# avi2924/Speech-Intent-Recognizer

Hardware: AMD Instinct MI355X
Metric: utterances/sec (16 kHz, 3 s clips), inference: HIP STFT+mel+CNN/BiGRU forward + argmax (higher is better)
Workload: dtype f32

## Files before the change

### speech-intent-recognizer_amd/csrc/conv_wino2_f16x3_kernel.h

```cpp
#pragma once
#include "conv_wino_bf16x6_kernel.h"
#include "wino2_geo.h"

constexpr int W2_RS = 11;
constexpr int W2_NPOS = 18 * W2_RS;
constexpr int W2_RAW_PIECES = (W2_NPOS * 4 + 63) / 64;
constexpr int W2_RAW_BYTES = W2_RAW_PIECES * 1024;
constexpr int W2_PLB = 16 * 1024;
constexpr int W2_NRAW = 3;
constexpr int W2_V_BYTES = 2 * W2_PLB;
constexpr int W2_XCH_BYTES = 3 * W2_PLB;
constexpr int W2_LDS_BYTES = 2 * W2_V_BYTES + W2_NRAW * W2_RAW_BYTES + W2_XCH_BYTES;
constexpr int W2_THREADS = 768;
constexpr int W2_PPW = (W2_RAW_PIECES + 3) / 4;

__device__ __forceinline__ int w2_div(int n, const W2Div& d) {
    const unsigned un = (unsigned)n;
    if (d.pow2) return (int)(un >> d.sh);
    const unsigned t = __umulhi(d.m, un);
    return (int)((t + ((un - t) >> 1)) >> d.sh);
}

__device__ __forceinline__ void split_w_f16x3(float u, unsigned short& p0, unsigned short& p1, unsigned int* status) {
    constexpr float LIM = 31.984375f;
// ... 8 lines not shown
                                                            unsigned int* status) {
    const int total = cin * 16 * cout;
    if (idx >= total) return;
    const int e = idx & 15, co = (idx >> 4) % cout, g = (idx >> 4) / cout;
    const int ci = (g / 16) * 16 + e, f = g % 16, i = f >> 2, j = f & 3;
    const float* gk = w + ((size_t)co * cin + ci) * 9;
    const float Gm[4][3] = {{1.f, 0.f, 0.f}, {.5f, .5f, .5f}, {.5f, -.5f, .5f}, {0.f, 0.f, 1.f}};
    float u = 0.0f;
#pragma unroll
    for (int k = 0; k < 3; ++k) {
        float t = 0.0f;
#pragma unroll
        for (int l = 0; l < 3; ++l) t = fmaf(gk[k * 3 + l], Gm[j][l], t);
        u = fmaf(Gm[i][k], t, u);
    }
    if (j == 3) u = -u;
    split_w_f16x3(u, wpb[idx], wpb[(size_t)total + idx], status);
}
#ifndef SIR_NO_STANDALONE_KERNELS
static __global__ void prep_conv_w_wino_f16x3_kernel(const float* __restrict__ w, unsigned short* __restrict__ wpb, int cin, int cout,
                                                     unsigned int* status) {
    prep_conv_w_wino_f16x3_elem(w, wpb, cin, cout, blockIdx.x * blockDim.x + threadIdx.x, status);
}
#endif
__device__ __forceinline__ void prep_conv_wT_wino_f16x3_elem(const float* __restrict__ w, unsigned short* __restrict__ wpb, int cin_f, int cout_f,
                                                             int idx, unsigned int* status) {
    const int total = cout_f * 16 * cin_f;
    if (idx >= total) return;
    const int e = idx & 15, cop = (idx >> 4) % cin_f, g = (idx >> 4) / cin_f;
    const int co_f = (g / 16) * 16 + e, f = g % 16, i = f >> 2, j = f & 3;
    const float* gk = w + ((size_t)co_f * cin_f + cop) * 9;
    const float Gm[4][3] = {{1.f, 0.f, 0.f}, {.5f, .5f, .5f}, {.5f, -.5f, .5f}, {0.f, 0.f, 1.f}};
    float u = 0.0f;
#pragma unroll
    for (int k = 0; k < 3; ++k) {
        float t = 0.0f;
#pragma unroll
        for (int l = 0; l < 3; ++l) t = fmaf(gk[8 - (k * 3 + l)], Gm[j][l], t);
        u = fmaf(Gm[i][k], t, u);
    }
    if (j == 3) u = -u;
    split_w_f16x3(u, wpb[idx], wpb[(size_t)total + idx], status);
}
#ifndef SIR_NO_STANDALONE_KERNELS
static __global__ void prep_conv_wT_wino_f16x3_kernel(const float* __restrict__ w, unsigned short* __restrict__ wpb, int cin_f, int cout_f,
                                                       unsigned int* status) {
    prep_conv_wT_wino_f16x3_elem(w, wpb, cin_f, cout_f, blockIdx.x * blockDim.x + threadIdx.x, status);
}
#endif

typedef float w2_f32x4 __attribute__((ext_vector_type(4)));
typedef unsigned w2_u32x2 __attribute__((ext_vector_type(2)));
__device__ __forceinline__ void w2_barrier() { asm volatile("s_waitcnt lgkmcnt(0)\n\ts_barrier" ::: "memory"); }
__device__ __forceinline__ void w2_read_row(unsigned base, w2_f32x4& r0, w2_f32x4& r1, w2_f32x4& r2, w2_f32x4& r3) {
    asm volatile("ds_read_b128 %0, %4\n\tds_read_b128 %1, %4 offset:64\n\tds_read_b128 %2, %4 offset:128\n\tds_read_b128 %3, %4 offset:192"
                 : "=&v"(r0), "=&v"(r1), "=&v"(r2), "=&v"(r3) : "v"(base) : "memory");
}
template <int OFF>
__device__ __forceinline__ void w2_write64(unsigned base, uint2 v) {
    const w2_u32x2 d = {v.x, v.y};
    asm volatile("ds_write_b64 %0, %1 offset:%2" :: "v"(base), "v"(d), "n"(OFF) : "memory");
}

__device__ long long w2_dbg_stamps[2][32];
__device__ long long w2_dbg_fine[8][8];
template <int CIN, int COUT, int OUT_MODE, int DBG = 0, int PRIO = 3, bool RAGGED = false>
__global__ __launch_bounds__(W2_THREADS, 3) void conv3x3_wino2_f16x3_kernel(
    const float* __restrict__ x, const unsigned short* __restrict__ wpb, const float* __restrict__ scale,
    const float* __restrict__ shift, float* __restrict__ out, Wino2Geo geo, float2* __restrict__ stats, const float* __restrict__ zeros) {
    constexpr int NCH = CIN / 16, G = NCH * 16, NCHO = COUT >= 64 ? COUT / 64 : 1;
    static_assert(CIN % 16 == 0 && (COUT % 64 == 0 || COUT == 32), "16-channel chunks; 64-channel tasks (32: the n = 1 consumer waves only keep the barriers)");
    static_assert(NCH >= 2, "a task's exchange pieces are read behind its closing barrier; the next task's are written >= one barrier later");
    extern __shared__ __attribute__((aligned(1024))) unsigned char w2s[];
    constexpr int VB = W2_V_BYTES;
    unsigned char* const vbuf = w2s;
    unsigned char* const rawbuf = w2s + 2 * VB;
    unsigned char* const xchbuf = rawbuf + W2_NRAW * W2_RAW_BYTES;

    const int tid = threadIdx.x, lane = tid & 63, wv = __builtin_amdgcn_readfirstlane(tid >> 6);
    const bool producer = wv < 4;
    const int H = geo.H, W = geo.W, TW = geo.TW, NG = geo.NG, RBN = geo.RBN;
    const int* const ctab = OUT_MODE <= 1 ? geo.ctab : nullptr;
    const int NS = ctab ? RBN * ctab[0] : geo.NS;
    const int ntask_s = (NS - (int)blockIdx.x + (int)gridDim.x - 1) / (int)gridDim.x;
    const int ntask = ntask_s * NCHO;
    if (ntask <= 0) return;
    const int nsteps = ntask * NCH;

    auto task_geo = [&](int lt, int& g0, int& ty0, int& ch, int& s) {
        s = (int)blockIdx.x + (lt / NCHO) * (int)gridDim.x;
        ch = lt % NCHO;
        const int cb = w2_div(s, geo.dRBN), rb = s - cb * RBN;
        g0 = ctab ? ctab[1 + cb] : 4 * cb; ty0 = 8 * rb;
    };
    constexpr bool IDLE_DMA = COUT < 64;
    constexpr int D_STRIDE = 4, D_PPW = (W2_RAW_PIECES + D_STRIDE - 1) / D_STRIDE;
    const int d_stride = D_STRIDE;
    const int d_rank = producer ? wv : ((wv - 4) >> 1);
    int pre_lr[D_PPW], pre_lc[D_PPW], pre_part[D_PPW];
#pragma unroll
    for (int ii = 0; ii < D_PPW; ++ii) {
        const int slot = 64 * (d_rank + d_stride * ii) + lane, pos = slot >> 2, sp = slot & 3;
        const int lr = pos / W2_RS;
        const int lc = pos - lr * W2_RS - ((lr >> 1) & 1);
        const bool hole = lr > 17 || lc < 0 || lc > 9;
        pre_lr[ii] = hole ? (1 << 20) : lr;
        pre_lc[ii] = lc;
        pre_part[ii] = (sp ^ (((lr >> 2) & 1) << 1)) * 4;
    }
    auto raw_offsets = [&](int g0, int ty0, unsigned (&off)[D_PPW]) {
        const int gimg = ctab ? w2_div(g0, geo.dTW) : 0;
        const int plo = ctab ? 2 * TW * gimg : 0, phi = ctab ? plo + (RAGGED ? min(W, geo.wtab[gimg] >> geo.wsh) : W) : 2 * NG;
#pragma unroll
        for (int ii = 0; ii < D_PPW; ++ii) {
            const int gy = 2 * ty0 - 1 + pre_lr[ii];
            const int P = 2 * g0 - 1 + pre_lc[ii];
            const int Pc = min(max(P, 0), 2 * NG - 1);
            const int bb = w2_div(Pc, geo.d2TW), px = Pc - bb * 2 * TW;
            const bool ok = gy >= 0 && gy < H && P >= plo && P < phi && px < W;
            off[ii] = ok ? (unsigned)(((bb * H + gy) * W + px) * CIN + pre_part[ii]) : ~0u;
        }
    };
        auto raw_issue = [&](const unsigned (&off)[D_PPW], int c, int slot_buf) {
#pragma unroll
        for (int ii = 0; ii < D_PPW; ++ii) {
            const int k = d_rank + d_stride * ii;
            if (k < W2_RAW_PIECES) {
                const float* src = off[ii] == ~0u ? zeros : x + off[ii];
                __builtin_amdgcn_global_load_lds((sir_gptr_t)(src + c * 16), (sir_lptr_t)(rawbuf + slot_buf * W2_RAW_BYTES + k * 1024), 16, 0, 0);
            }
        }
    };
    int ig0, ity0, ich, is_;
    unsigned roff[D_PPW];
    int roff_task = -1;
    auto issue_chunk = [&](int q) {
        if (q >= nsteps) return;
        const int lt = q / NCH, c = q - lt * NCH;
        if (lt != roff_task) { task_geo(lt, ig0, ity0, ich, is_); raw_offsets(ig0, ity0, roff); roff_task = lt; }
        raw_issue(roff, c, q % W2_NRAW);
    };
    int nst = 0;
    auto stamp = [&]() {
        if (DBG && blockIdx.x == 0 && lane == 0 && (wv == 0 || wv == 4) && nst < 32) w2_dbg_stamps[producer ? 0 : 1][nst] = __builtin_amdgcn_s_memtime();
        ++nst;
    };

    if (producer) {
        if (PRIO) __builtin_amdgcn_s_setprio(PRIO);
        __builtin_amdgcn_s_setreg((1 ) | (23 << 6) | (0 << 11), 1);
        const int wg = wv;
        const int tR = wg >> 1, tH = wg & 1, tm = lane >> 1, tP1 = lane & 1;
        const int tty = tm & 7, ttx = tm >> 3, tpart = 2 * tH + tP1;
        unsigned ra_rel[3];
#pragma unroll
        for (int rr = 0; rr < 3; ++rr) {
            const int lr = 2 * tty + tR + rr;
            ra_rel[rr] = (unsigned)((lr * W2_RS + 2 * ttx + ((lr >> 1) & 1)) * 64 + ((tpart ^ (((lr >> 2) & 1) << 1)) * 16));
        }
        const unsigned raw_a = (unsigned)(uintptr_t)rawbuf, v_a = (unsigned)(uintptr_t)vbuf + (8 * tR) * 1024 + tH * 512 + tm * 16 + tP1 * 8;
        if (!IDLE_DMA) {
            issue_chunk(0);
            issue_chunk(1);
            asm volatile("s_waitcnt vmcnt(0)" ::: "memory");
        }
        w2_barrier();
        bool edge = false, z0 = false, z3 = false;
        auto fine = [&](int s_, int k_) {
            if (DBG && blockIdx.x == 0 && lane == 0 && wv == 0 && s_ >= 8 && s_ < 16) w2_dbg_fine[s_ - 8][k_] = __builtin_amdgcn_s_memtime();
        };
#pragma unroll 1
        for (int s = 0; s <= nsteps; ++s) {
            stamp();
            fine(s, 0);
            if (s < nsteps) {
                if (!IDLE_DMA && !(DBG & 2)) issue_chunk(s + 2);
                fine(s, 1);
                if (s % NCH == 0) {
                    int cg0, cty0, cch, cs;
                    task_geo(s / NCH, cg0, cty0, cch, cs);
                    const int t0 = cg0 - w2_div(cg0, geo.dTW) * TW;
                    edge = !ctab && (t0 == 0 || t0 + 3 >= TW - 1);
                    const int txx = (t0 + ttx) - w2_div(t0 + ttx, geo.dTW) * TW;
                    z0 = txx == 0; z3 = txx == TW - 1;
                }
                const unsigned rb = raw_a + (s % W2_NRAW) * W2_RAW_BYTES, vd = v_a + (s & 1) * VB;
                if (!(DBG & 4)) {
                w2_f32x4 q[3][4];
#pragma unroll
                for (int rr = 0; rr < 3; ++rr) w2_read_row(rb + ra_rel[rr], q[rr][0], q[rr][1], q[rr][2], q[rr][3]);
                asm volatile("s_waitcnt lgkmcnt(0)" ::: "memory");
                fine(s, 2);
                if (edge) {
                    asm volatile("" ::: "memory");
                    const w2_f32x4 zero4 = {0.0f, 0.0f, 0.0f, 0.0f};
#pragma unroll
                    for (int rr = 0; rr < 3; ++rr) { q[rr][0] = z0 ? zero4 : q[rr][0]; q[rr][3] = z3 ? zero4 : q[rr][3]; }
                }
                auto rows = [&](auto trc) {
                    constexpr int TR = decltype(trc)::value;
#pragma unroll
                    for (int il = 0; il < 2; ++il) {
                        w2_f32x4 R[4];
#pragma unroll
                        for (int j = 0; j < 4; ++j) {
                            if (TR == 0) R[j] = il == 0 ? q[0][j] - q[2][j] : q[1][j] + q[2][j];
                            else         R[j] = il == 0 ? q[1][j] - q[0][j] : q[0][j] - q[2][j];
                        }
                        const w2_f32x4 V[4] = {R[0] - R[2], R[1] + R[2], R[2] - R[1], R[1] - R[3]};
#pragma unroll
                        for (int j = 0; j < 4; ++j) {
                            const unsigned d = vd + (4 * il + j) * 1024;
                            uint2 sh, sl;
                            split2h_pair_ovfl(V[j].x, V[j].y, sh.x, sl.x);
                            split2h_pair_ovfl(V[j].z, V[j].w, sh.y, sl.y);
                            w2_write64<0>(d, sh);
                            w2_write64<W2_PLB>(d, sl);
                        }
                    }
                };
                if (tR == 0) rows(std::integral_constant<int, 0>{});
                else rows(std::integral_constant<int, 1>{});
                if (DBG) asm volatile("s_waitcnt lgkmcnt(0)" ::: "memory");
                fine(s, 3);
                }
                if (!IDLE_DMA) {
                    if (s + 2 < nsteps) asm volatile("s_waitcnt vmcnt(%0)" :: "n"(W2_RAW_PIECES / 4) : "memory");
                    else asm volatile("s_waitcnt vmcnt(0)" ::: "memory");
                }
            }
            stamp();
            fine(s, 4);
            w2_barrier();
            fine(s, 5);
        }
        return;
    }

    const int cw = wv - 4, mn = cw & 1, mi = cw >> 1, m = lane & 31, h = lane >> 5;
    if (COUT < 64 && mn == 1) {
        if (IDLE_DMA) {
            if (!(DBG & 2)) { issue_chunk(0); issue_chunk(1); }
            asm volatile("s_waitcnt vmcnt(0)" ::: "memory");
            w2_barrier();
#pragma unroll 1
            for (int s = 0; s <= nsteps; ++s) {
                if (s < nsteps) {
                    if (!(DBG & 2)) issue_chunk(s + 2);
                    if (s + 2 < nsteps) asm volatile("s_waitcnt vmcnt(%0)" :: "n"(W2_RAW_PIECES / 4) : "memory");
                    else asm volatile("s_waitcnt vmcnt(0)" ::: "memory");
                }
                w2_barrier();
            }
            return;
        }
        w2_barrier();
        w2_barrier();
        for (int lt = 0; lt < ntask; ++lt)
            for (int c = 0; c < NCH; ++c) w2_barrier();
        return;
    }
    const unsigned wlane = (unsigned)((m * 2 + h) * 16);
    const unsigned char* const wbase = reinterpret_cast<const unsigned char*>(wpb) + (size_t)mn * 1024;
    constexpr int NPW = 2;
    uint4 wq[4][NPW];
    auto load_w = [&](int gidx, int chh, uint4 (&q)[NPW]) {
#pragma unroll
        for (int p = 0; p < NPW; ++p)
            q[p] = *reinterpret_cast<const uint4*>(wbase + ((size_t)(p * G + gidx) * (COUT * 2) + (size_t)chh * 128) * 16 + wlane);
    };
    int g0, ty0, ch, s_idx;
    task_geo(0, g0, ty0, ch, s_idx);
#pragma unroll
    for (int j = 0; j < 4; ++j) load_w(4 * mi + j, ch, wq[j]);
    f32x16 acc[4];
#pragma unroll
    for (int j = 0; j < 4; ++j)
#pragma unroll
        for (int r = 0; r < 16; ++r) acc[j][r] = 0.0f;
    w2_barrier();
    float run_s[NCHO], run_q[NCHO];
#pragma unroll
    for (int k = 0; k < NCHO; ++k) { run_s[k] = 0.0f; run_q[k] = 0.0f; }

    stamp();
    stamp();
    w2_barrier();
#pragma unroll 1
    for (int lt = 0; lt < ntask; ++lt) {
        int g0n = g0, ty0n = ty0, chn = ch, sn = s_idx;
        if (lt + 1 < ntask) task_geo(lt + 1, g0n, ty0n, chn, sn);
#pragma unroll 1
        for (int c = 0; c < NCH; ++c) {
            stamp();
            const int sc = lt * NCH + c;
            const bool task_end = c == NCH - 1;
            const unsigned char* abase = vbuf + (sc & 1) * VB + h * 512 + m * 16 + (4 * mi) * 1024;
            const int gnxt = (task_end ? 0 : c + 1) * 16 + 4 * mi;
#pragma unroll
            for (int jp = 0; jp < 2; ++jp) {
                constexpr int NPA = 2;
                bf16x8 a[2][NPA], bq[2][3];
#pragma unroll
                for (int jj = 0; jj < 2; ++jj) {
#pragma unroll
                    for (int p = 0; p < NPA; ++p)
                        a[jj][p] = __builtin_bit_cast(bf16x8, *reinterpret_cast<const uint4*>(abase + p * W2_PLB + (2 * jp + jj) * 1024));
                    const f16x8 uh = __builtin_bit_cast(f16x8, wq[2 * jp + jj][0]);
                    bq[jj][0] = __builtin_bit_cast(bf16x8, uh);
                    bq[jj][1] = __builtin_bit_cast(bf16x8, uh * (_Float16)2048.0f);
                    bq[jj][2] = __builtin_bit_cast(bf16x8, wq[2 * jp + jj][1]);
                }
                if (DBG & 8) {
#pragma unroll
                    for (int jj = 0; jj < 2; ++jj)
                        acc[2 * jp + jj][0] += __builtin_bit_cast(float4, a[jj][0]).x + __builtin_bit_cast(float4, a[jj][1]).y + __builtin_bit_cast(float4, a[jj][NPA - 1]).z +
                                               __builtin_bit_cast(float4, bq[jj][0]).x + __builtin_bit_cast(float4, bq[jj][1]).y + __builtin_bit_cast(float4, bq[jj][2]).z;
                } else {
                    constexpr int HA[3] = {1, 0, 0}, HB[3] = {0, 2, 1};
#pragma unroll
                    for (int t3 = 0; t3 < 3; ++t3)
#pragma unroll
                        for (int jj = 0; jj < 2; ++jj)
                            acc[2 * jp + jj] = __builtin_amdgcn_mfma_f32_32x32x16_f16(__builtin_bit_cast(f16x8, a[jj][HA[t3]]),
                                                                                      __builtin_bit_cast(f16x8, bq[jj][HB[t3]]), acc[2 * jp + jj], 0, 0, 0);
                }
#pragma unroll
                for (int jj = 0; jj < 2; ++jj) if (!(DBG & 64)) load_w(gnxt + 2 * jp + jj, task_end ? chn : ch, wq[2 * jp + jj]);
                __builtin_amdgcn_sched_barrier(0);
            }
            stamp();
            if (!task_end) w2_barrier();
        }
        if (DBG & 16) { w2_barrier(); if (acc[0][0] == 1234.5f && acc[1][1] + acc[2][2] + acc[3][3] == 4.0f) out[0] = 1.0f; }
        else {
            {
                float4* const xch = reinterpret_cast<float4*>(xchbuf);
                float own[2][4];
#pragma unroll
                for (int b = 0; b < 2; ++b) {
                    const f32x16 Wc = b == 0 ? acc[0] + acc[1] + acc[2] : acc[1] - acc[2] + acc[3];
#pragma unroll
                    for (int k = 0; k < 4; ++k) {
                        if (k == mi) {
#pragma unroll
                            for (int e = 0; e < 4; ++e) own[b][e] = Wc[4 * k + e];
                        } else {
                            float4* dst = xch + (size_t)((mn * 4 + mi) * 3 + ((k - mi - 1) & 3)) * 128 + lane;
                            dst[b * 64] = make_float4(Wc[4 * k], Wc[4 * k + 1], Wc[4 * k + 2], Wc[4 * k + 3]);
                        }
                    }
                }
                w2_barrier();
                float Y[2][2][4];
#pragma unroll
                for (int i = 0; i < 4; ++i) {
                    const int kk = (mi - i - 1) & 3;
                    const float4* src = xch + (size_t)((mn * 4 + i) * 3 + (kk < 3 ? kk : 0)) * 128 + lane;
#pragma unroll
                    for (int b = 0; b < 2; ++b) {
                        const float4 v = src[b * 64];
                        const float w[4] = {i == mi ? own[b][0] : v.x, i == mi ? own[b][1] : v.y, i == mi ? own[b][2] : v.z, i == mi ? own[b][3] : v.w};
#pragma unroll
                        for (int e = 0; e < 4; ++e) {
                            if (i == 0) Y[0][b][e] = w[e];
                            else if (i <= 2) Y[0][b][e] += w[e];
                            if (i == 1) Y[1][b][e] = w[e];
                            else if (i >= 2) Y[1][b][e] -= w[e];
                        }
                    }
                }
                const int co = ch * 64 + mn * 32 + m;
                float ssum = 0.0f, ssq = 0.0f;
                float sc_ = 1.0f, sh_ = 0.0f;
                constexpr float DESC = H3_LO_INV;
                if (OUT_MODE <= 1) { sc_ = scale[co] * DESC; sh_ = shift[co]; }
                {
                    const int gc = g0 + mi;
                    const int img = w2_div(gc, geo.dTW), tx = gc - img * TW;
                    const bool tvalid = gc < (ctab ? (w2_div(g0, geo.dTW) + 1) * TW : NG);
                    const int wpi = RAGGED ? min(geo.Wp, geo.wtab[w2_div(g0, geo.dTW)] >> (geo.wsh + 1)) : geo.Wp;
                    if (OUT_MODE <= 1) {
                        float pooled[4];
#pragma unroll
                        for (int e = 0; e < 4; ++e) {
                            float v = 0.0f;
#pragma unroll
                            for (int a = 0; a < 2; ++a)
#pragma unroll
                                for (int b = 0; b < 2; ++b) v = fmaxf(v, fmaf(Y[a][b][e], sc_, sh_));
                            pooled[e] = v;
                        }
                        if (tvalid && tx < wpi) {
                            if (OUT_MODE == 0) {
#pragma unroll
                                for (int e = 0; e < 4; ++e)
                                    out[(((size_t)img * geo.Hp + ty0 + 4 * h + e) * geo.Wp + tx) * COUT + co] = pooled[e];
                            } else {
                                const size_t oidx = ((size_t)img * geo.Wp + tx) * (COUT * geo.Hp) + (size_t)co * geo.Hp + ty0 + 4 * h;
                                const float4 v4 = make_float4(pooled[0], pooled[1], pooled[2], pooled[3]);
                                *reinterpret_cast<float4*>(out + oidx) = v4;
                                if (stats) {
                                    unsigned short* planes = reinterpret_cast<unsigned short*>(stats);
                                    const size_t plane = (size_t)geo.B * geo.Wp * (COUT * geo.Hp);
                                    uint2 hh, ll;
                                    split2h_quad(v4, hh, ll);
                                    *reinterpret_cast<uint2*>(planes + oidx) = hh;
                                    *reinterpret_cast<uint2*>(planes + plane + oidx) = ll;
                                }
                            }
                        }
                    } else {
#pragma unroll
                        for (int e = 0; e < 4; ++e)
#pragma unroll
                            for (int a = 0; a < 2; ++a)
#pragma unroll
                                for (int b = 0; b < 2; ++b) {
                                    const int gy = 2 * (ty0 + 4 * h + e) + a, gx = 2 * tx + b;
                                    if (tvalid && gx < W) {
                                        const float v = Y[a][b][e] * DESC;
                                        out[(((size_t)img * H + gy) * W + gx) * COUT + co] = v;
                                        ssum += v;
                                        ssq = fmaf(v, v, ssq);
                                    }
                                }
                    }
                }
                if (OUT_MODE == 2) {
#pragma unroll
                    for (int k = 0; k < NCHO; ++k)
                        if (k == ch) { run_s[k] += ssum; run_q[k] += ssq; }
                }
            }
        }
        g0 = g0n; ty0 = ty0n; ch = chn; s_idx = sn;
#pragma unroll
        for (int j = 0; j < 4; ++j)
#pragma unroll
            for (int r = 0; r < 16; ++r) acc[j][r] = 0.0f;
    }
    if (OUT_MODE == 2 && stats) {
#pragma unroll
        for (int k = 0; k < NCHO; ++k) {
            float a = run_s[k], q = run_q[k];
            a += __shfl_xor(a, 32);
            q += __shfl_xor(q, 32);
            if (h == 0) stats[((size_t)blockIdx.x * 4 + mi) * COUT + k * 64 + mn * 32 + m] = make_float2(a, q);
        }
    }
}

template <int CIN, int COUT, int OUT_MODE, int DBG = 0, int PRIO = 3, bool RAGGED = false>
static inline hipError_t launch_conv_wino2(hipStream_t st, Wino2Geo g, const float* x, const unsigned short* wpb, const float* scale,
                                           const float* shift, float* out, float2* stats, const float* zeros, int max_wg = 256,
                                           const int* ctab = nullptr, int ncol_max = 0, const int* wtab = nullptr, int wsh = 0) {
    if (RAGGED && (!ctab || !wtab)) return hipErrorInvalidValue;
    g.wtab = wtab; g.wsh = wsh;
    if (ctab) {
        if (OUT_MODE > 1 || ncol_max < 1) return hipErrorInvalidValue;
        g.ctab = ctab;
        g.NS = g.RBN * ncol_max;
    }
    const int nwg = g.NS < max_wg ? g.NS : max_wg;
    hipLaunchKernelGGL((conv3x3_wino2_f16x3_kernel<CIN, COUT, OUT_MODE, DBG, PRIO, RAGGED>), dim3(nwg), dim3(W2_THREADS), W2_LDS_BYTES, st, x, wpb, scale, shift, out, g, stats, zeros);
    return hipGetLastError();
}
```

### speech-intent-recognizer_amd/csrc/model_infer.hip

```cpp
#include "f16x3_kernels.h"
#include "conv_fwd.h"
#include "gru_frag_prep.h"

namespace {

enum WsBuf {
    WS_A1 = 0,
    WS_A2,
    WS_X0,
    WS_GI,
    WS_Y0,
    WS_Y1,
    WS_CTX,
    WS_PAD,
    WS_XZ,
    WS_BN,
    WS_WHT,
    WS_XS,
    WS_WS,
    WS_WCB,
    WS_GXB,
    WS_GFL,
    WS_COUNT
};

struct Dims : SirDims {
    int tw2, tw3, k2max, k3max;
};

bool make_dims(int batch, int t_frames, Dims* d) {
    if (!sir_make_dims(batch, t_frames, d)) return false;
    d->tw2 = (d->wp1 + 1) / 2; d->tw3 = (d->wp2 + 1) / 2; d->k2max = (d->tw2 + 3) / 4; d->k3max = (d->tw3 + 3) / 4;
    return true;
}

struct PadTabs { size_t e0, d1, d3, tab2, tab3, rows, count; };
PadTabs pad_tabs(const Dims& d) {
    PadTabs t;
    const size_t n = (size_t)d.B + 1;
    t.e0 = 0; t.d1 = d.B; t.d3 = t.d1 + n; t.tab2 = t.d3 + n; t.tab3 = t.tab2 + 1 + n * d.k2max; t.rows = t.tab3 + 1 + n * d.k3max;
    t.count = t.rows + 1 + n * d.S;
    return t;
}

void ws_sizes(const Dims& d, size_t* bytes) {
    const size_t B = d.B + 1;
    bytes[WS_A1] = B * 32 * d.wp1 * 32 * 4;
    bytes[WS_A2] = B * 16 * d.wp2 * 64 * 4;
    bytes[WS_X0] = B * d.S * 1024 * 4;
    bytes[WS_GI] = B * d.S * 1536 * 4;
    bytes[WS_Y0] = (size_t)d.B * d.S * 512 * 4;
    bytes[WS_Y1] = (size_t)d.B * d.S * 512 * 4;
    bytes[WS_CTX] = (size_t)d.B * 512 * 4;
    bytes[WS_PAD] = pad_tabs(d).count * 4;
    bytes[WS_XZ] = (size_t)64 * d.T * 4;
    bytes[WS_BN] = (size_t)2 * 224 * 4;
    bytes[WS_WHT] = 4 * GRU_FRAG_BYTES;
    bytes[WS_XS] = B * d.S * 1024 * 2 * 2;
    bytes[WS_WS] = ((size_t)2 * 2 * 768 * 1024 + (size_t)2 * 2 * 768 * 512) * 2;
    bytes[WS_WCB] = ((size_t)3 * 32 * 16 * 64 + (size_t)3 * 64 * 16 * 128 + (size_t)3 * 64 * 9 * 128) * 2;
    bytes[WS_GXB] = 0;
    bytes[WS_GFL] = 0;
}

size_t ws_layout(const Dims& d, size_t* off) {
    size_t bytes[WS_COUNT], pos = 0;
    ws_sizes(d, bytes);
    for (int i = 0; i < WS_COUNT; ++i) {
        off[i] = pos;
        pos += sir_align_up(bytes[i], 256);
    }
    return pos;
}

static __global__ __launch_bounds__(256) void pad_extent_kernel(const float* __restrict__ x, int T, int* __restrict__ e0) {
    const unsigned* xb = reinterpret_cast<const unsigned*>(x) + (size_t)blockIdx.x * 64 * T;
    int last = -1;
    for (int c = threadIdx.x; c < T; c += 256) {
        unsigned acc = 0;
#pragma unroll 32
        for (int r = 0; r < 64; ++r) acc |= xb[(size_t)r * T + c];
        if (acc) last = c;
    }
#pragma unroll
    for (int o = 32; o > 0; o >>= 1) last = max(last, __shfl_xor(last, o));
    __shared__ int wl[4];
    if ((threadIdx.x & 63) == 0) wl[threadIdx.x >> 6] = last;
    __syncthreads();
    if (threadIdx.x == 0) e0[blockIdx.x] = max(max(wl[0], wl[1]), max(wl[2], wl[3])) + 1;
}

template <typename Need>
__device__ __forceinline__ void pad_tables_emit(const Dims& d, int nu, Need need, int* __restrict__ d1o, int* __restrict__ d3o,
                                                int* __restrict__ tab2, int* __restrict__ tab3, int* __restrict__ prow) {
    const int tid = threadIdx.x;
    const int per = (nu + 1023) / 1024, u0 = min(nu, tid * per), u1 = min(nu, u0 + per);
    int s2 = 0, s3 = 0, sr = 0, c1, c3, k2, k3;
    for (int u = u0; u < u1; ++u) { need(u, c1, c3, k2, k3); s2 += k2; s3 += k3; sr += c3; }
    __shared__ int p2[1024], p3[1024], pr[1024];
    p2[tid] = s2; p3[tid] = s3; pr[tid] = sr;
    __syncthreads();
    for (int o = 1; o < 1024; o <<= 1) {
        const int a2 = tid >= o ? p2[tid - o] : 0, a3 = tid >= o ? p3[tid - o] : 0, ar = tid >= o ? pr[tid - o] : 0;
        __syncthreads();
        p2[tid] += a2; p3[tid] += a3; pr[tid] += ar;
        __syncthreads();
    }
    int o2 = p2[tid] - s2, o3 = p3[tid] - s3, orw = pr[tid] - sr;
    for (int u = u0; u < u1; ++u) {
        need(u, c1, c3, k2, k3);
        d1o[u] = c1; d3o[u] = c3;
        for (int k = 0; k < k2; ++k) tab2[1 + o2 + k] = u * d.tw2 + 4 * k;
        for (int k = 0; k < k3; ++k) tab3[1 + o3 + k] = u * d.tw3 + 4 * k;
        for (int s = 0; s < c3; ++s) prow[1 + orw + s] = u * d.S + s;
        o2 += k2; o3 += k3; orw += c3;
    }
    if (tid == 1023) { tab2[0] = p2[1023]; tab3[0] = p3[1023]; prow[0] = pr[1023]; }
}

static __global__ __launch_bounds__(1024) void pad_tables_kernel(const int* __restrict__ e0, Dims d, int* __restrict__ d1o, int* __restrict__ d3o,
                                                                 int* __restrict__ tab2, int* __restrict__ tab3, int* __restrict__ prow,
                                                                 float* __restrict__ xz) {
    const int tid = threadIdx.x;
    for (int i = tid; i < 64 * d.T; i += 1024) xz[i] = 0.0f;
    auto need = [&](int u, int& c1, int& c3, int& k2, int& k3) {
        if (u == d.B) { c1 = d.wp1; c3 = d.S; k2 = d.k2max; k3 = d.k3max; return; }
        c3 = min(d.S, (e0[u] + 14) / 8);
        const int c2 = min(d.wp2, 2 * c3 + 1);
        c1 = min(d.wp1, 2 * c2 + 1);
        k2 = (c2 + 3) / 4; k3 = (c3 + 3) / 4;
    };
    pad_tables_emit(d, d.B + 1, need, d1o, d3o, tab2, tab3, prow);
}

static __global__ __launch_bounds__(1024) void ragged_tables_kernel(const int* __restrict__ frames, Dims d, int* __restrict__ fw, int* __restrict__ d1o,
                                                                    int* __restrict__ d3o, int* __restrict__ tab2, int* __restrict__ tab3,
                                                                    int* __restrict__ prow, unsigned int* __restrict__ status) {
    bool bad = false;
    for (int u = threadIdx.x; u < d.B; u += 1024) {
        const int f0 = frames[u], f = f0 >= 8 && f0 <= d.T ? f0 : 0;
        fw[u] = f;
        bad |= f == 0;
    }
    if (bad) __hip_atomic_fetch_or(status, 64u, __ATOMIC_RELAXED, __HIP_MEMORY_SCOPE_AGENT);
    __syncthreads();
    auto need = [&](int u, int& c1, int& c3, int& k2, int& k3) {
        const int f = fw[u];
        c1 = f >> 1; c3 = f >> 3;
        k2 = ((f >> 2) + 3) / 4; k3 = (c3 + 3) / 4;
    };
    pad_tables_emit(d, d.B, need, d1o, d3o, tab2, tab3, prow);
}

static __global__ __launch_bounds__(256) void ragged_mask_kernel(float* __restrict__ a, const int* __restrict__ fw, int sh, int H, int W, int C) {
    const int b = blockIdx.y, r = blockIdx.x, w0 = min(W, fw[b] >> sh);
    float4* row = reinterpret_cast<float4*>(a + (((size_t)b * H + r) * W + w0) * C);
    const int n4 = (W - w0) * (C / 4);
    for (int i = threadIdx.x; i < n4; i += 256) row[i] = make_float4(0.0f, 0.0f, 0.0f, 0.0f);
}

}

extern "C" size_t sir_model_workspace_bytes(const sir_handle* h, int batch, int t_frames, int train) {
    (void)h;
    if (train) return sir_train_workspace_bytes_impl(batch, t_frames);
    Dims d;
    if (!make_dims(batch, t_frames, &d)) return 0;
    size_t off[WS_COUNT];
    return ws_layout(d, off);
}

extern "C" int sir_model_workspace_offsets(const sir_handle* h, int batch, int t_frames, int train, size_t* offsets,
                                           int n) {
    (void)h; (void)train;
    Dims d;
    if (!make_dims(batch, t_frames, &d) || !offsets) { sir_set_error("sir_model_workspace_offsets: bad shape"); return SIR_EINVAL; }
    size_t off[WS_COUNT];
    ws_layout(d, off);
    for (int i = 0; i < n && i < WS_COUNT; ++i) offsets[i] = off[i];
    return WS_COUNT;
}

static int model_infer_impl(const char* who, sir_handle* h, const sir_model_weights* w, const float* feats, const int32_t* frames, int batch,
                            int t_frames, float* logits, int64_t* argmax, void* workspace, size_t workspace_bytes, void* stream_) {
    if (!h || !w || !feats || !logits || !workspace) { sir_set_error("%s: NULL argument", who); return SIR_EINVAL; }
    Dims d;
    if (!make_dims(batch, t_frames, &d)) {
        sir_set_error("%s: unsupported shape batch=%d t_frames=%d (need t_frames >= 8)", who, batch, t_frames);
        return SIR_EINVAL;
    }
    if (h->cfg.n_mels != 64) { sir_set_error("%s: the model is wired for 64 mels (models.py:23)", who); return SIR_EUNSUPPORTED; }
    if (w->num_classes < 1 || w->num_classes > 64) { sir_set_error("%s: num_classes=%d", who, w->num_classes); return SIR_EINVAL; }
    size_t off[WS_COUNT];
    const size_t need = ws_layout(d, off);
    if (workspace_bytes < need) { sir_set_error("%s: workspace %zu < %zu", who, workspace_bytes, need); return SIR_ENOMEM; }
    if (((uintptr_t)workspace & 255) != 0) { sir_set_error("%s: workspace must be 256-byte aligned", who); return SIR_EINVAL; }
    const bool ragged = frames != nullptr;
    hipStream_t st = (hipStream_t)stream_;
    char* ws = (char*)workspace;
    float* a1 = (float*)(ws + off[WS_A1]);
    float* a2 = (float*)(ws + off[WS_A2]);
    float* x0 = (float*)(ws + off[WS_X0]);
    float* gi = (float*)(ws + off[WS_GI]);
    float* y0 = (float*)(ws + off[WS_Y0]);
    float* y1 = (float*)(ws + off[WS_Y1]);
    float* ctx = (float*)(ws + off[WS_CTX]);
    float* bns = (float*)(ws + off[WS_BN]);
    float* bnt = bns + 224;
    float* wht = (float*)(ws + off[WS_WHT]);
    unsigned short* xs = (unsigned short*)(ws + off[WS_XS]);
    unsigned short* wsl0 = (unsigned short*)(ws + off[WS_WS]);
    unsigned short* wsl1 = wsl0 + (size_t)2 * 2 * 768 * 1024;
    unsigned short* wcb2 = (unsigned short*)(ws + off[WS_WCB]);
    unsigned short* wcb3 = wcb2 + (size_t)3 * 32 * 16 * 64;
    unsigned short* wcb3d = wcb3 + (size_t)3 * 64 * 16 * 128;
    const int B = d.B, S = d.S;
    const PadTabs pt = pad_tabs(d);
    int* const ptab = (int*)(ws + off[WS_PAD]);
    float* const xz = (float*)(ws + off[WS_XZ]);

    const SirConvPlan cp = sir_conv_plan(&d, true);
    const bool w2 = cp.fwd_wino;
    const int BT = w2 ? B + 1 : B;

    const long long prep_key = ((long long)B << 32) | (unsigned)d.T;
    sir_handle::PrepEntry* pe = nullptr;
    for (auto& e : h->prep)
        if (e.ws == workspace) pe = &e;
    const bool reuse_prep = pe && h->weights_version != 0 && pe->version == h->weights_version && pe->key == prep_key;
    if (!reuse_prep) {
        SirProfScope prof(h, SIR_K_PREP, st);
        const int bn_c[3] = {32, 64, 128}, bn_o[3] = {0, 32, 96};
        for (int i = 0; i < 3; ++i)
            hipLaunchKernelGGL(prep_bn_kernel, dim3(1), dim3(128), 0, st, w->bn_w[i], w->bn_b[i], w->bn_mean[i], w->bn_var[i],
// ... 112 lines not shown
```

### speech-intent-recognizer_amd/ops.py

```python
import ctypes as C
import itertools

import torch

from . import _native
from .featurizer import get_featurizer

GRU_SUFFIXES = ("_l0", "_l0_reverse", "_l1", "_l1_reverse")
WS_NAMES = ("conv1", "conv2", "gru_in", "gi", "gru_l0", "gru_l1", "ctx")


def _f32c(t, name):
    if t.dtype != torch.float32 or not t.is_contiguous():
        raise _native.SirError(f"{name} must be contiguous float32")
    if not t.is_cuda:
        raise _native.SirError(f"{name} is not on a HIP device (no CPU fallback)")
    return t


def weights_struct(mod):
    w = _native.ModelWeights()
    keep = []

    def p(t, name):
# ... 78 lines not shown
        if rc == _native.SIR_OK and int(flag.item()):
            raise _native.SirError("sir_check_status failed on another rank of this job (a GRU recurrence timed out or a "
                                   "label was out of range there): this rank stops with it")
    _native.check(rc, "sir_check_status")


def _as_features(x):
    if x.dim() == 4:
        if x.shape[1] != 1:
            raise _native.SirError("input_channels must be 1")
        x = x[:, 0]
    if x.dim() != 3 or x.shape[1] != 64:
        raise _native.SirError(f"expected [B,64,T] or [B,1,64,T], got {tuple(x.shape)}")
    if x.shape[2] < 8:
        raise _native.SirError("need at least 8 frames")
    return _f32c(x.contiguous(), "input")


def _as_lengths(lengths, bsz, t, device):
    if not torch.is_tensor(lengths):
        lengths = torch.as_tensor(list(lengths))
    if lengths.dim() != 1 or lengths.numel() != bsz:
        raise _native.SirError(f"lengths must hold one entry per clip: got shape {tuple(lengths.shape)} for a batch of {bsz}")
    if lengths.is_floating_point() or lengths.dtype == torch.bool:
        raise _native.SirError("lengths must be integers (frames per clip)")
    if not lengths.is_cuda:
        bad = [(i, int(v)) for i, v in enumerate(lengths.tolist()) if not 8 <= int(v) <= t]
        if bad:
            raise _native.SirError(f"lengths outside [8, {t}] (clip, frames): {bad[:8]}")
        lengths = lengths.to(device)
    return lengths.to(torch.int32).contiguous()


def model_infer(mod, x, workspace, want_argmax=False, debug=None, lengths=None):
    _native.require_hip(x)
    x = _as_features(x)
    bsz, _, t = x.shape
    lib = _native.lib()
    h = get_featurizer().handle
    need = lib.sir_model_workspace_bytes(h, bsz, t, 0)
    if need == 0:
        raise _native.SirError(f"unsupported shape batch={bsz} frames={t}")
    if lengths is not None:
        lengths = _as_lengths(lengths, bsz, t, x.device)
    ws = workspace.get(need, x.device)
    w, keep = cached_weights(mod)
    logits = torch.empty((bsz, w.num_classes), dtype=torch.float32, device=x.device)
    amax = torch.empty((bsz,), dtype=torch.int64, device=x.device) if want_argmax else None
    lib.sir_model_set_weights_version(h, weights_version(mod, keep, workspace))
    if lengths is None:
        rc = lib.sir_model_infer(h, C.byref(w), x.data_ptr(), bsz, t, logits.data_ptr(),
                                 amax.data_ptr() if amax is not None else None, ws.data_ptr(), ws.numel(),
                                 _native.current_stream_ptr())
        _native.check(rc, "sir_model_infer")
    else:
        rc = lib.sir_model_infer_ragged(h, C.byref(w), x.data_ptr(), lengths.data_ptr(), bsz, t, logits.data_ptr(),
                                        amax.data_ptr() if amax is not None else None, ws.data_ptr(), ws.numel(),
                                        _native.current_stream_ptr())
        _native.check(rc, "sir_model_infer_ragged")
    if debug is not None:
        debug.update(stage_views(ws, bsz, t))
    del keep
    return (logits, amax) if want_argmax else logits


def stage_views(ws, bsz, t):
    lib = _native.lib()
    offs = (C.c_size_t * 16)()
    n = lib.sir_model_workspace_offsets(get_featurizer().handle, bsz, t, 0, offs, 16)
    if n <= 0:
        raise _native.SirError("sir_model_workspace_offsets failed")
    wp1, wp2 = t // 2, t // 4
    s = wp2 // 2
    shapes = {"conv1": (bsz, 32, wp1, 32), "conv2": (bsz, 16, wp2, 64), "gru_in": (bsz, s, 1024),
              "gi": (bsz * s, 1536), "gru_l0": (bsz, s, 512), "gru_l1": (bsz, s, 512), "ctx": (bsz, 512)}
    out = {}
    for i, name in enumerate(WS_NAMES):
        shp = shapes[name]
        numel = 1
        for v in shp:
            numel *= v
        out[name] = ws[offs[i]: offs[i] + 4 * numel].view(torch.float32).view(shp)
    return out
```

Baseline: 724,600.

## Pack ragged column-block tails into guest slots and rebalance output-channel task dealing

```diff
diff --git a/speech-intent-recognizer_amd/csrc/conv_wino2_f16x3_kernel.h b/speech-intent-recognizer_amd/csrc/conv_wino2_f16x3_kernel.h
--- a/speech-intent-recognizer_amd/csrc/conv_wino2_f16x3_kernel.h
+++ b/speech-intent-recognizer_amd/csrc/conv_wino2_f16x3_kernel.h
@@ -114,16 +114,30 @@
     const int H = geo.H, W = geo.W, TW = geo.TW, NG = geo.NG, RBN = geo.RBN;
     const int* const ctab = OUT_MODE <= 1 ? geo.ctab : nullptr;
     const int NS = ctab ? RBN * ctab[0] : geo.NS;
-    const int ntask_s = (NS - (int)blockIdx.x + (int)gridDim.x - 1) / (int)gridDim.x;
-    const int ntask = ntask_s * NCHO;
+    constexpr bool HALF_DEAL = OUT_MODE <= 1 && NCHO > 1;
+    const int GD = (int)gridDim.x, bx = (int)blockIdx.x;
+    const int nfull = HALF_DEAL ? NS / GD : 0;
+    const int nfull_t = nfull * NCHO;
+    const int ntask = HALF_DEAL ? nfull_t + ((NS - nfull * GD) * NCHO - bx + GD - 1) / GD : ((NS - bx + GD - 1) / GD) * NCHO;
     if (ntask <= 0) return;
     const int nsteps = ntask * NCH;
 
-    auto task_geo = [&](int lt, int& g0, int& ty0, int& ch, int& s) {
-        s = (int)blockIdx.x + (lt / NCHO) * (int)gridDim.x;
-        ch = lt % NCHO;
+    auto task_geo = [&](int lt, int& g0, int& na, int& bw, int& ty0, int& ch, int& s) {
+        if (HALF_DEAL && lt >= nfull_t) {
+            const int r = bx + (lt - nfull_t) * GD;
+            s = nfull * GD + r / NCHO;
+            ch = r % NCHO;
+        } else {
+            s = bx + (lt / NCHO) * GD;
+            ch = lt % NCHO;
+        }
         const int cb = w2_div(s, geo.dRBN), rb = s - cb * RBN;
-        g0 = ctab ? ctab[1 + cb] : 4 * cb; ty0 = 8 * rb;
+        const int2 tw = ctab ? reinterpret_cast<const int2*>(ctab)[1 + cb] : make_int2((4 * cb) << 2 | 3, -1);
+        g0 = tw.x >> 2; na = 1 + (tw.x & 3); bw = RAGGED ? -1 : tw.y; ty0 = 8 * rb;
+    };
+    auto guest_geo = [&](int g0, int bw, int& sB, int& gB, int& nB) {
+        const bool guest = bw >= 0;
+        sB = guest ? 2 + ((bw >> 1) & 1) : 8; gB = guest ? bw >> 2 : g0; nB = guest ? 1 + (bw & 1) : 0;
     };
     constexpr bool IDLE_DMA = COUT < 64;
     constexpr int D_STRIDE = 4, D_PPW = (W2_RAW_PIECES + D_STRIDE - 1) / D_STRIDE;
@@ -140,13 +154,19 @@
         pre_lc[ii] = lc;
         pre_part[ii] = (sp ^ (((lr >> 2) & 1) << 1)) * 4;
     }
-    auto raw_offsets = [&](int g0, int ty0, unsigned (&off)[D_PPW]) {
-        const int gimg = ctab ? w2_div(g0, geo.dTW) : 0;
-        const int plo = ctab ? 2 * TW * gimg : 0, phi = ctab ? plo + (RAGGED ? min(W, geo.wtab[gimg] >> geo.wsh) : W) : 2 * NG;
+    auto raw_offsets = [&](int g0, int bw, int ty0, unsigned (&off)[D_PPW]) {
+        int sB, gB, nB;
+        guest_geo(g0, bw, sB, gB, nB);
+        const int gimg = ctab ? w2_div(g0, geo.dTW) : 0, gimgB = ctab ? w2_div(gB, geo.dTW) : 0;
+        const int ploA = ctab ? 2 * TW * gimg : 0, phiA = ctab ? ploA + (RAGGED ? min(W, geo.wtab[gimg] >> geo.wsh) : W) : 2 * NG;
+        const int ploB = 2 * TW * gimgB, phiB = ploB + W;
+        const int cA = 2 * g0 - 1, cB = 2 * (gB - sB) - 1, lcB = 2 * sB;
 #pragma unroll
         for (int ii = 0; ii < D_PPW; ++ii) {
             const int gy = 2 * ty0 - 1 + pre_lr[ii];
-            const int P = 2 * g0 - 1 + pre_lc[ii];
+            const bool inB = pre_lc[ii] >= lcB;
+            const int plo = inB ? ploB : ploA, phi = inB ? phiB : phiA;
+            const int P = (inB ? cB : cA) + pre_lc[ii];
             const int Pc = min(max(P, 0), 2 * NG - 1);
             const int bb = w2_div(Pc, geo.d2TW), px = Pc - bb * 2 * TW;
             const bool ok = gy >= 0 && gy < H && P >= plo && P < phi && px < W;
@@ -163,13 +183,13 @@
             }
         }
     };
-    int ig0, ity0, ich, is_;
+    int ig0, ina, ibw, ity0, ich, is_;
     unsigned roff[D_PPW];
     int roff_task = -1;
     auto issue_chunk = [&](int q) {
         if (q >= nsteps) return;
         const int lt = q / NCH, c = q - lt * NCH;
-        if (lt != roff_task) { task_geo(lt, ig0, ity0, ich, is_); raw_offsets(ig0, ity0, roff); roff_task = lt; }
+        if (lt != roff_task) { task_geo(lt, ig0, ina, ibw, ity0, ich, is_); raw_offsets(ig0, ibw, ity0, roff); roff_task = lt; }
         raw_issue(roff, c, q % W2_NRAW);
     };
     int nst = 0;
@@ -208,9 +228,9 @@
             if (s < nsteps) {
                 if (!IDLE_DMA && !(DBG & 2)) issue_chunk(s + 2);
                 fine(s, 1);
-                if (s % NCH == 0) {
-                    int cg0, cty0, cch, cs;
-                    task_geo(s / NCH, cg0, cty0, cch, cs);
+                if (s % NCH == 0 && !ctab) {
+                    int cg0, cna, cbw, cty0, cch, cs;
+                    task_geo(s / NCH, cg0, cna, cbw, cty0, cch, cs);
                     const int t0 = cg0 - w2_div(cg0, geo.dTW) * TW;
                     edge = !ctab && (t0 == 0 || t0 + 3 >= TW - 1);
                     const int txx = (t0 + ttx) - w2_div(t0 + ttx, geo.dTW) * TW;
@@ -301,8 +321,8 @@
         for (int p = 0; p < NPW; ++p)
             q[p] = *reinterpret_cast<const uint4*>(wbase + ((size_t)(p * G + gidx) * (COUT * 2) + (size_t)chh * 128) * 16 + wlane);
     };
-    int g0, ty0, ch, s_idx;
-    task_geo(0, g0, ty0, ch, s_idx);
+    int g0, na, bw, ty0, ch, s_idx;
+    task_geo(0, g0, na, bw, ty0, ch, s_idx);
 #pragma unroll
     for (int j = 0; j < 4; ++j) load_w(4 * mi + j, ch, wq[j]);
     f32x16 acc[4];
@@ -320,8 +340,8 @@
     w2_barrier();
 #pragma unroll 1
     for (int lt = 0; lt < ntask; ++lt) {
-        int g0n = g0, ty0n = ty0, chn = ch, sn = s_idx;
-        if (lt + 1 < ntask) task_geo(lt + 1, g0n, ty0n, chn, sn);
+        int g0n = g0, nan_ = na, bwn = bw, ty0n = ty0, chn = ch, sn = s_idx;
+        if (lt + 1 < ntask) task_geo(lt + 1, g0n, nan_, bwn, ty0n, chn, sn);
 #pragma unroll 1
         for (int c = 0; c < NCH; ++c) {
             stamp();
@@ -408,10 +428,14 @@
                 constexpr float DESC = H3_LO_INV;
                 if (OUT_MODE <= 1) { sc_ = scale[co] * DESC; sh_ = shift[co]; }
                 {
-                    const int gc = g0 + mi;
+                    int sB, gB, nB;
+                    guest_geo(g0, bw, sB, gB, nB);
+                    const bool inB = mi >= sB;
+                    const int sfirst = inB ? gB : g0, sk = inB ? mi - sB : mi, scnt = inB ? nB : na;
+                    const int gc = sfirst + sk, img0 = w2_div(sfirst, geo.dTW);
                     const int img = w2_div(gc, geo.dTW), tx = gc - img * TW;
-                    const bool tvalid = gc < (ctab ? (w2_div(g0, geo.dTW) + 1) * TW : NG);
-                    const int wpi = RAGGED ? min(geo.Wp, geo.wtab[w2_div(g0, geo.dTW)] >> (geo.wsh + 1)) : geo.Wp;
+                    const bool tvalid = sk < scnt && gc < (ctab ? (img0 + 1) * TW : NG);
+                    const int wpi = RAGGED ? min(geo.Wp, geo.wtab[img0] >> (geo.wsh + 1)) : geo.Wp;
                     if (OUT_MODE <= 1) {
                         float pooled[4];
 #pragma unroll
@@ -466,7 +490,7 @@
                 }
             }
         }
-        g0 = g0n; ty0 = ty0n; ch = chn; s_idx = sn;
+        g0 = g0n; na = nan_; bw = bwn; ty0 = ty0n; ch = chn; s_idx = sn;
 #pragma unroll
         for (int j = 0; j < 4; ++j)
 #pragma unroll
diff --git a/speech-intent-recognizer_amd/csrc/model_infer.hip b/speech-intent-recognizer_amd/csrc/model_infer.hip
--- a/speech-intent-recognizer_amd/csrc/model_infer.hip
+++ b/speech-intent-recognizer_amd/csrc/model_infer.hip
@@ -38,8 +38,10 @@
 PadTabs pad_tabs(const Dims& d) {
     PadTabs t;
     const size_t n = (size_t)d.B + 1;
-    t.e0 = 0; t.d1 = d.B; t.d3 = t.d1 + n; t.tab2 = t.d3 + n; t.tab3 = t.tab2 + 1 + n * d.k2max; t.rows = t.tab3 + 1 + n * d.k3max;
-    t.count = t.rows + 1 + n * d.S;
+    t.e0 = 0; t.d1 = d.B; t.d3 = t.d1 + n; t.rows = t.d3 + n + 1 + n * d.k2max + 1 + n * d.k3max;
+    t.tab2 = t.rows + 1 + n * d.S; t.tab2 += t.tab2 & 1;
+    t.tab3 = t.tab2 + 2 + 2 * n * d.k2max;
+    t.count = t.tab3 + 2 + 2 * n * d.k3max;
     return t;
 }
 
@@ -90,32 +92,99 @@
     if (threadIdx.x == 0) e0[blockIdx.x] = max(max(wl[0], wl[1]), max(wl[2], wl[3])) + 1;
 }
 
-template <typename Need>
+__device__ __forceinline__ int pk_cap(int r) { const int l = r & 3; return l == 1 ? 2 : l == 2 ? 1 : 0; }
+__device__ __forceinline__ int pk_take(int c, int g, int cn) { return g <= c ? min(pk_cap(c - g), cn) : 0; }
+constexpr int PK_ID = 0 | 1 << 2 | 2 << 4;
+__device__ __forceinline__ int pk_fn(int c, int cn) { return pk_take(c, 0, cn) | pk_take(c, 1, cn) << 2 | pk_take(c, 2, cn) << 4; }
+__device__ __forceinline__ int pk_then(int f, int g) {
+    int r = 0;
+#pragma unroll
+    for (int x = 0; x < 3; ++x) r |= ((g >> (2 * ((f >> (2 * x)) & 3))) & 3) << (2 * x);
+    return r;
+}
+__device__ __forceinline__ void pk_emit(int* __restrict__ tab, int o, int base, int g, int r, int gB, int nB) {
+    const int k = (r + 3) >> 2;
+    for (int t = 0; t < k; ++t) {
+        reinterpret_cast<int2*>(tab)[1 + o + t] = make_int2((base + g + 4 * t) << 2 | (min(4, r - 4 * t) - 1),
+                                                            t == k - 1 && nB > 0 ? gB << 2 | (2 - nB) << 1 | (nB - 1) : -1);
+    }
+}
+
+template <bool PACK, typename Need>
 __device__ __forceinline__ void pad_tables_emit(const Dims& d, int nu, Need need, int* __restrict__ d1o, int* __restrict__ d3o,
                                                 int* __restrict__ tab2, int* __restrict__ tab3, int* __restrict__ prow) {
     const int tid = threadIdx.x;
     const int per = (nu + 1023) / 1024, u0 = min(nu, tid * per), u1 = min(nu, u0 + per);
-    int s2 = 0, s3 = 0, sr = 0, c1, c3, k2, k3;
-    for (int u = u0; u < u1; ++u) { need(u, c1, c3, k2, k3); s2 += k2; s3 += k3; sr += c3; }
-    __shared__ int p2[1024], p3[1024], pr[1024];
-    p2[tid] = s2; p3[tid] = s3; pr[tid] = sr;
-    __syncthreads();
-    for (int o = 1; o < 1024; o <<= 1) {
-        const int a2 = tid >= o ? p2[tid - o] : 0, a3 = tid >= o ? p3[tid - o] : 0, ar = tid >= o ? pr[tid - o] : 0;
+    const int nr = PACK ? nu - 1 : nu;
+    __shared__ int wt[3][16];
+    auto scan = [&](auto op, int id, int& a, int& b, int& c, int& ta, int& tb, int& tc) {
+        const int ln = tid & 63, wv = tid >> 6;
+#pragma unroll
+        for (int o = 1; o < 64; o <<= 1) {
+            const int xa = __shfl_up(a, o), xb = __shfl_up(b, o), xc = __shfl_up(c, o);
+            if (ln >= o) { a = op(xa, a); b = op(xb, b); c = op(xc, c); }
+        }
         __syncthreads();
-        p2[tid] += a2; p3[tid] += a3; pr[tid] += ar;
+        if (ln == 63) { wt[0][wv] = a; wt[1][wv] = b; wt[2][wv] = c; }
         __syncthreads();
-    }
-    int o2 = p2[tid] - s2, o3 = p3[tid] - s3, orw = pr[tid] - sr;
-    for (int u = u0; u < u1; ++u) {
-        need(u, c1, c3, k2, k3);
-        d1o[u] = c1; d3o[u] = c3;
-        for (int k = 0; k < k2; ++k) tab2[1 + o2 + k] = u * d.tw2 + 4 * k;
-        for (int k = 0; k < k3; ++k) tab3[1 + o3 + k] = u * d.tw3 + 4 * k;
-        for (int s = 0; s < c3; ++s) prow[1 + orw + s] = u * d.S + s;
-        o2 += k2; o3 += k3; orw += c3;
-    }
-    if (tid == 1023) { tab2[0] = p2[1023]; tab3[0] = p3[1023]; prow[0] = pr[1023]; }
+        int pa = id, pb = id, pc = id;
+        ta = id; tb = id; tc = id;
+        for (int w = 0; w < 16; ++w) {
+            const int va = wt[0][w], vb = wt[1][w], vc = wt[2][w];
+            if (w < wv) { pa = op(pa, va); pb = op(pb, vb); pc = op(pc, vc); }
+            ta = op(ta, va); tb = op(tb, vb); tc = op(tc, vc);
+        }
+        const int xa = __shfl_up(a, 1), xb = __shfl_up(b, 1), xc = __shfl_up(c, 1);
+        a = ln ? op(pa, xa) : pa; b = ln ? op(pb, xb) : pb; c = ln ? op(pc, xc) : pc;
+    };
+    auto add = [](int a, int b) { return a + b; };
+    int c1, c2, c3, n1, n2, n3;
+    int q2_0 = 0, q3_0 = 0, orw0 = 0, cap2, cap3, nrow;
+    for (int u = u0; u < u1; ++u) { need(u, c1, c2, c3); orw0 += c3; if (PACK && u < nr) { q2_0 += pk_cap(c2); q3_0 += pk_cap(c3); } }
+    scan(add, 0, q2_0, q3_0, orw0, cap2, cap3, nrow);
+    int t2 = 0, t3 = 0, gt2 = 0, gt3 = 0;
+    if (PACK) { need(nr, c1, t2, t3); gt2 = min(t2, cap2); gt3 = min(t3, cap3); }
+    int g2 = 0, g3 = 0;
+    if (PACK) {
+        int f2 = PK_ID, f3 = PK_ID, fx = PK_ID, q2 = q2_0, q3 = q3_0, x2, x3, xx;
+        for (int u = u0; u < min(u1, nr); ++u) {
+            need(u, c1, c2, c3);
+            n2 = n3 = 0;
+            if (u + 1 < nr) need(u + 1, n1, n2, n3);
+            f2 = pk_then(f2, q2 < t2 ? 0 : pk_fn(c2, n2)); f3 = pk_then(f3, q3 < t3 ? 0 : pk_fn(c3, n3));
+            q2 += pk_cap(c2); q3 += pk_cap(c3);
+        }
+        scan([](int a, int b) { return pk_then(a, b); }, PK_ID, f2, f3, fx, x2, x3, xx);
+        g2 = f2 & 3; g3 = f3 & 3;
+    }
+    auto walk = [&](bool emit, int& o2, int& o3, int orw) {
+        int q2 = q2_0, q3 = q3_0, h2 = g2, h3 = g3;
+        for (int u = u0; u < u1; ++u) {
+            need(u, c1, c2, c3);
+            int b2 = 0, b3 = 0, m2 = 0, m3 = 0, x2 = 0, x3 = 0;
+            if (PACK && u < nr) {
+                n2 = n3 = 0;
+                if (u + 1 < nr) need(u + 1, n1, n2, n3);
+                if (q2 < t2) { b2 = nr * d.tw2 + q2; m2 = min(pk_cap(c2), t2 - q2); } else { b2 = (u + 1) * d.tw2; m2 = x2 = pk_take(c2, h2, n2); }
+                if (q3 < t3) { b3 = nr * d.tw3 + q3; m3 = min(pk_cap(c3), t3 - q3); } else { b3 = (u + 1) * d.tw3; m3 = x3 = pk_take(c3, h3, n3); }
+                q2 += pk_cap(c2); q3 += pk_cap(c3);
+            } else if (PACK) { h2 = gt2; h3 = gt3; }
+            const int r2 = c2 - h2, r3 = c3 - h3;
+            if (emit) {
+                d1o[u] = c1; d3o[u] = c3;
+                pk_emit(tab2, o2, u * d.tw2, h2, r2, b2, m2);
+                pk_emit(tab3, o3, u * d.tw3, h3, r3, b3, m3);
+                for (int s = 0; s < c3; ++s) prow[1 + orw + s] = u * d.S + s;
+            }
+            o2 += (r2 + 3) >> 2; o3 += (r3 + 3) >> 2; orw += c3;
+            h2 = x2; h3 = x3;
+        }
+    };
+    int o2 = 0, o3 = 0, ox = 0, nt2, nt3, ntx;
+    walk(false, o2, o3, 0);
+    scan(add, 0, o2, o3, ox, nt2, nt3, ntx);
+    walk(true, o2, o3, orw0);
+    if (tid == 0) { tab2[0] = nt2; tab3[0] = nt3; prow[0] = nrow; }
 }
 
 static __global__ __launch_bounds__(1024) void pad_tables_kernel(const int* __restrict__ e0, Dims d, int* __restrict__ d1o, int* __restrict__ d3o,
@@ -123,14 +192,13 @@
                                                                  float* __restrict__ xz) {
     const int tid = threadIdx.x;
     for (int i = tid; i < 64 * d.T; i += 1024) xz[i] = 0.0f;
-    auto need = [&](int u, int& c1, int& c3, int& k2, int& k3) {
-        if (u == d.B) { c1 = d.wp1; c3 = d.S; k2 = d.k2max; k3 = d.k3max; return; }
+    auto need = [&](int u, int& c1, int& c2, int& c3) {
+        if (u == d.B) { c1 = d.wp1; c2 = d.wp2; c3 = d.S; return; }
         c3 = min(d.S, (e0[u] + 14) / 8);
-        const int c2 = min(d.wp2, 2 * c3 + 1);
+        c2 = min(d.wp2, 2 * c3 + 1);
         c1 = min(d.wp1, 2 * c2 + 1);
-        k2 = (c2 + 3) / 4; k3 = (c3 + 3) / 4;
     };
-    pad_tables_emit(d, d.B + 1, need, d1o, d3o, tab2, tab3, prow);
+    pad_tables_emit<true>(d, d.B + 1, need, d1o, d3o, tab2, tab3, prow);
 }
 
 static __global__ __launch_bounds__(1024) void ragged_tables_kernel(const int* __restrict__ frames, Dims d, int* __restrict__ fw, int* __restrict__ d1o,
@@ -144,12 +212,11 @@
     }
     if (bad) __hip_atomic_fetch_or(status, 64u, __ATOMIC_RELAXED, __HIP_MEMORY_SCOPE_AGENT);
     __syncthreads();
-    auto need = [&](int u, int& c1, int& c3, int& k2, int& k3) {
+    auto need = [&](int u, int& c1, int& c2, int& c3) {
         const int f = fw[u];
-        c1 = f >> 1; c3 = f >> 3;
-        k2 = ((f >> 2) + 3) / 4; k3 = (c3 + 3) / 4;
+        c1 = f >> 1; c2 = f >> 2; c3 = f >> 3;
     };
-    pad_tables_emit(d, d.B, need, d1o, d3o, tab2, tab3, prow);
+    pad_tables_emit<false>(d, d.B, need, d1o, d3o, tab2, tab3, prow);
 }
 
 static __global__ __launch_bounds__(256) void ragged_mask_kernel(float* __restrict__ a, const int* __restrict__ fw, int sh, int H, int W, int C) {
diff --git a/speech-intent-recognizer_amd/ops.py b/speech-intent-recognizer_amd/ops.py
--- a/speech-intent-recognizer_amd/ops.py
+++ b/speech-intent-recognizer_amd/ops.py
@@ -184,3 +184,25 @@
             numel *= v
         out[name] = ws[offs[i]: offs[i] + 4 * numel].view(torch.float32).view(shp)
     return out
+
+
+def pad_skip_tables(ws, bsz, t):
+    lib = _native.lib()
+    offs = (C.c_size_t * 16)()
+    if lib.sir_model_workspace_offsets(get_featurizer().handle, bsz, t, 0, offs, 16) <= 7:
+        raise _native.SirError("sir_model_workspace_offsets failed")
+    wp1, wp2 = t // 2, t // 4
+    k2max, k3max = ((wp1 + 1) // 2 + 3) // 4, ((wp2 + 1) // 2 + 3) // 4
+    n = bsz + 1
+    o_d3 = bsz + n
+    o_rows = o_d3 + n + 1 + n * k2max + 1 + n * k3max
+    o_tab2 = o_rows + 1 + n * (wp2 // 2)
+    o_tab2 += o_tab2 & 1
+    o_tab3 = o_tab2 + 2 + 2 * n * k2max
+    o_end = o_tab3 + 2 + 2 * n * k3max
+    tab = ws[offs[7]: offs[7] + 4 * o_end].view(torch.int32).cpu()
+    out = {"e0": tab[:bsz], "d3": tab[o_d3: o_d3 + n]}
+    for name, o in (("tab2", o_tab2), ("tab3", o_tab3)):
+        cnt = int(tab[o])
+        out[name] = tab[o + 2: o + 2 + 2 * cnt].view(cnt, 2)
+    return out
```

After: 752,700 (median of 6 runs). 1.04x the previous value.
